# NomaDamas/AutoRAG-Research

Hardware: AMD Instinct MI355X
Metric: queries/sec (higher is better)
Workload: dtype f32

## Files before the change

autorag_research_amd/csrc/index.h:

```cpp
#pragma once
#include <climits>
#include <hip/hip_runtime.h>

#include <algorithm>
#include <cmath>
#include <cstdio>
#include <cstring>
#include <mutex>
#include <string>
#include <vector>

#include "dev_common.h"
#include "mi355dr.h"

namespace mi355 {
template <class T, bool Pinned = false>
struct DevBuf {
    T* p = nullptr;
    size_t bytes = 0;
    DevBuf() = default;
    DevBuf(const DevBuf&) = delete;
    DevBuf& operator=(const DevBuf&) = delete;
    ~DevBuf() { release(); }
    void release() {
// ... 27 lines not shown
    Event& operator=(const Event&) = delete;
    ~Event() {
        if (e) (void)hipEventDestroy(e);
    }
    hipError_t create(unsigned flags = hipEventDefault) { return e ? hipSuccess : hipEventCreateWithFlags(&e, flags); }
    operator hipEvent_t() const { return e; }
};

struct EventPair {
    hipEvent_t a, b;
    int big;
};
struct EventPairs {
    std::vector<EventPair> v;
    ~EventPairs() {
        for (auto& p : v) {
            (void)hipEventDestroy(p.a);
            (void)hipEventDestroy(p.b);
        }
    }
};
struct MultiVecStore;
struct SparseStore;
struct Pass {
    int k = 0;
    int level = 0;
    bool screening = false;
    bool i8 = false;
    bool wide = false;
    int cap = 0;
    bool speculative = false;
    bool spec_eligible = false;
    int spec_m = 0;
    const char* refused = nullptr;
};
struct Pending {
    bool active = false;
    Event done;
    HostBuf<int> status_host;
    hipStream_t stream = nullptr;
    const float* q_dev = nullptr;
    int B = 0;
    Pass pass;
    double* out_dist = nullptr;
    int64_t* out_rows = nullptr;
};
struct RetryBufs {
    DevBuf<float> q;
    DevBuf<double> dist;
    DevBuf<int64_t> rows;
    DevBuf<int> map;
};
constexpr int kPendingRing = 4;

template <class... Bufs>
hipError_t grow_each(size_t n, Bufs&... bufs) {
    hipError_t e = hipSuccess;
    (void)(((e = bufs.grow(n * sizeof(*bufs.p))) == hipSuccess) && ...);
    return e;
}
struct MmrBufs {
    DevBuf<double> cand_dist;
    DevBuf<int64_t> cand_rows;
    DevBuf<unsigned long long> pairs_dev;
    hipError_t reserve(size_t nb, size_t stride) {
        hipError_t e = grow_each(nb * stride, cand_dist, cand_rows);
// ... 134 lines not shown
    int speculate = 1;
    int64_t spec_min_rows = (int64_t)1 << 20;
    int spec_shift_milli = 0;
    int spec_backoff = 0, spec_probation = 0;
    mi355::DevBuf<float> spec_moments;
    int i8_demoted_k = INT_MAX;
    double i8_min_budget = 0.25;
    mi355::RetryBufs retry[3];
    mi355::Pending pend[mi355::kPendingRing];
    mi355::Pending sub_pend[4];
    int64_t seq_next = 0, seq_done = 0;
    int last_pass_k = 10;
    int maxsim_coop = -1;
    int maxsim_persistent = 0;
    int maxsim_wg = -1;
    int maxsim_tighten = 1;
    int maxsim_aligned = 1;
    int maxsim_wg_min = 8;
    int maxsim_wg_pipe = 1;
    int maxsim_pack8 = -1;
    int maxsim_wg_bps = 4;
    int maxsim_pass_groups = 4;
    int maxsim_screen = 1;
    int maxsim_subset_screen = -1;
    int64_t maxsim_subset_screen_min = 512;
    int64_t row_offset = 0;
    int round_a = 0;
    int screen_rq = 1;
    int screen_stream = 1;
    int prefilter16 = 0;
    int profile = 0;
    int starter = 1;
    int prune_companion = 1;
    int scan_dma = 1;
    int defer_round_b = 1;
    int chunk0_set = 0;
    int64_t chunk0_rows = 1024;
    int64_t chunk_growth = 3;
    int chunk_growth_set = 0;
    int64_t small_chunk_rows = 16384;
    int cap = mi355::kCandCap;
    int cap_set = 0;
    int prune_wide = 1;
    int screen_flush_sync = 1, screen_flush_lanes = 48, screen_flush_alone = 40;
    int wide_inflation_x10 = 100;
    int chunk_taper_x100 = 0;
    int64_t compact_slice_rows = 65536;
    int64_t view_slice_rows = 65536;
    int64_t range_chunk_rows = (int64_t)1 << 21;
    int range_slots = mi355::kSortMax;
    int64_t shard_stage_bytes = (int64_t)256 << 20;
    int64_t starter_rows_wide = 65536;

    int64_t s_screen_launches = 0, s_screen_ns = 0, s_screen_rows = 0, s_fallback_queries = 0, s_chunks = 0,
            s_passes = 0, s_starters = 0;
    int64_t s_big_launches = 0, s_big_ns = 0, s_big_rows = 0;
    int screen_rq_split_tests = 1;
    int64_t debug_park = 0;
    mi355::DevBuf<float> park_thr;
    int screen_drift = 3;
    mi355::DevBuf<int> rq_progress;
    int rq_epoch = 0;
    int64_t s_rq_launches = 0;
    int64_t s_spec_passes = 0, s_spec_miss_queries = 0, s_spec_overflow_queries = 0;
    int64_t s_retry_queries = 0;
    int64_t s_ms_screened = 0, s_ms_candidates = 0, s_ms_fallbacks = 0;
    int64_t s_ms_screen_ns = 0, s_ms_screen_launches = 0, s_ms_exact_ns = 0, s_ms_exact_launches = 0, s_ms_pack_ns = 0;
    int64_t s_ms_packed_launches = 0;
    int64_t s_ms_packed_blocks = 0;
    int64_t s_ms_packed_built = 0;
    int64_t s_ms_set_docs = 0;
    int64_t s_ms_moved_blocks = 0;
    int64_t s_compactions = 0;
    int64_t s_compact_moved_rows = 0;
    int64_t s_subset_searches = 0;
    int64_t s_subset_rows_scored = 0;
    int64_t s_subset_rerun_queries = 0;
    int64_t s_mss_searches = 0, s_mss_docs = 0, s_mss_screened = 0, s_mss_exact = 0, s_mss_fallbacks = 0;
    int64_t s_mmr_searches = 0, s_mmr_queries = 0, s_mmr_pairs = 0;
    int64_t s_group_searches = 0, s_group_subqueries = 0, s_groups_merged = 0;
    int64_t s_fuse_calls = 0, s_fuse_queries = 0;
    int64_t s_range_searches = 0, s_range_queries = 0, s_range_in_range = 0, s_range_candidates = 0, s_range_rescored = 0,
            s_range_redo_chunks = 0, s_range_fallback_queries = 0;
    int64_t s_rows_searches = 0, s_rows_queries = 0, s_rows_skipped = 0;
    int64_t s_shard_range_searches = 0, s_shard_rows_searches = 0, s_shard_mmr_searches = 0, s_shard_gather_bytes = 0;
    int64_t s_shard_sparse_searches = 0, s_shard_sparse_scores = 0;
    int64_t s_sparse_searches = 0, s_sparse_queries = 0, s_sparse_postings_scored = 0, s_sparse_overflows = 0;
    int sparse_tile_docs = 2048;
    int sparse_cand_cap = 2048;
    int64_t sparse_subset_pairs_max = 2048;
    int64_t s_sparse_subset_searches = 0, s_sparse_subset_scores = 0, s_sparse_subset_pairs = 0, s_sparse_subset_tiles = 0;
    int sparse_overlay_max_pct = 25;
    int64_t s_sparse_full_builds = 0, s_sparse_overlay_builds = 0, s_sparse_sets = 0;
// ... 88 lines not shown
```

autorag_research_amd/csrc/k_select.h:

```cpp
#pragma once
#include "dev_common.h"

namespace mi355 {

struct PruneArgs {
    const float* rows;
    const float* nrm2;
    const float* q;
    QueryState st;
    int32_t* cand_row;
    float* cand_val;
    const int* qlist;
    unsigned long long* stat;
    int cap, d, k, metric;
    int exact;
    const uint8_t* flag8;
    float cscale;
    const uint16_t* shadow16;
    int dpad;
    int round_a;
    int* skip_list;
    int skip_parity;
    int thr_only;
    int one_wave_only;
    int defer_b;
    SpecModel spec;
};

__device__ __forceinline__ float unit_sim(int metric, double dist, float inv_qn) {
    return metric == 0 ? (float)(1.0 - dist) : (float)(-dist) * inv_qn;
}
__device__ __forceinline__ float screen_threshold(int metric, double dist_k, float E, float nq) {
    if (metric == 0) return float_below((float)((1.0 - dist_k) - (double)E));
    const double u = -dist_k / sqrt((double)nq);
    return float_below((float)(u - fabs(u) * 4e-6 - (double)E));
}

constexpr int kPruneSmallThreads = 64, kPruneSmallSort = 1024;
constexpr int kPruneBigThreads = 256, kPruneBigSort = kSortMax;

__host__ __device__ inline size_t prune_qs_floats(int d) { return ((size_t)d + 3) / 4 * 4 + 16; }
__host__ __device__ inline size_t prune_lds_bytes(int d, int threads, int sortmax, int dpad16) {
    size_t x = (size_t)(threads / kWave) * kStageFloats * sizeof(float);
    size_t lf = (size_t)sortmax * sizeof(float);
    if (lf > x) x = lf;
    return (size_t)sortmax * 8 + (size_t)sortmax * 4 + x + (size_t)sortmax * 4 + prune_qs_floats(d) * 4 + (size_t)dpad16 * 4;
}

template <int PER, int T, bool ROWS = false>
__device__ __forceinline__ void load_candidate_keys(uint32_t (&key)[PER], const float* __restrict__ cval,
                                                    const int32_t* __restrict__ crow, const uint8_t* __restrict__ flag8,
                                                    int n_new, int tid, int32_t* rows_out = nullptr) {
    float v[PER];
    int32_t r[PER];
    const int last = n_new - 1;
#pragma unroll
    for (int j = 0; j < PER; ++j) {
        v[j] = 0.0f;
        r[j] = 0;
        if (j * T >= n_new) continue;
// ... 23 lines not shown
        if (j * T + tid < n_new) {
            if (v[j] != v[j]) kk = 0xFFFFFFFFu;
            else if (!f[j]) kk = f32_order_key(v[j]);
        }
        key[j] = kk;
        if (ROWS) rows_out[j] = r[j];
    }
}

template <int THREADS, int SORT>
__device__ __forceinline__ void prune_body(const PruneArgs& a, char* smem);

template <int THREADS, int SORT>
__global__ __launch_bounds__(THREADS) void k_prune(PruneArgs a) {
    extern __shared__ __attribute__((aligned(16))) char smem[];
    const bool list_mode = a.skip_list != nullptr && a.qlist == nullptr;
    const int tid = threadIdx.x;
    const int lane = tid & 63, wave = tid >> 6;
    int q = a.qlist ? a.qlist[blockIdx.x] : blockIdx.x;
    if (SORT == kPruneBigSort && list_mode) {
        if (blockIdx.x == 0 && tid == 0) a.skip_list[a.skip_parity ^ 1] = 0;
        const int n_left = a.skip_list[a.skip_parity];
        for (int i = blockIdx.x; i < n_left; i += gridDim.x) {
            PruneArgs b = a;
            b.skip_list = nullptr;
            b.qlist = a.skip_list + 2 + a.skip_parity * kQBlockMax + i - 0;
            b.qlist -= blockIdx.x;
            prune_body<THREADS, SORT>(b, smem);
            __syncthreads();
        }
        return;
    }
    prune_body<THREADS, SORT>(a, smem);
}

template <int THREADS, int SORT>
__device__ __forceinline__ void prune_body(const PruneArgs& a, char* smem) {
    constexpr int kWaves = THREADS / kWave;
    uint64_t* SK = (uint64_t*)smem;
    int32_t* SR = (int32_t*)(smem + (size_t)SORT * 8);
    char* X = smem + (size_t)SORT * 12;
    constexpr size_t xa = (size_t)kWaves * kStageFloats * sizeof(float), xb = (size_t)SORT * sizeof(float);
    constexpr size_t xbytes = xa > xb ? xa : xb;
    float* Lf = (float*)X;
    float* tiles = (float*)X;
    int32_t* R = (int32_t*)(X + xbytes);
    float* qs = (float*)(X + xbytes + (size_t)SORT * 4);
    int& s_cnt = *(int*)(X + xbytes + (size_t)SORT * 4 + (prune_qs_floats(a.d) - 16) * 4);
    float* q16 = qs + prune_qs_floats(a.d);
    const bool list_mode = a.skip_list != nullptr && a.qlist == nullptr;
    const int q = a.qlist ? a.qlist[blockIdx.x] : blockIdx.x;
    const int tid = threadIdx.x;
    const int lane = tid & 63, wave = tid >> 6;
    const int raw_cnt = a.st.cnt[q];
    const int n_best = a.st.best_n[q];
    if (raw_cnt == 0) return;
    if (a.exact && SORT < kPruneBigSort) return;
    auto leave_for_general = [&]() {
        if (a.one_wave_only) {
            if (tid == 0) {
                a.st.status[q] |= kStOverflow;
                a.st.cnt[q] = 0;
            }
            return;
        }
        if (list_mode && tid == 0) {
            const int i = atomicAdd(&a.skip_list[a.skip_parity], 1);
            a.skip_list[2 + a.skip_parity * kQBlockMax + i] = q;
        }
    };
    if (raw_cnt > a.cap) {
        if (SORT < kPruneBigSort) {
            leave_for_general();
            return;
        }
        if (tid == 0) {
            a.st.status[q] |= kStOverflow;
            a.st.cnt[q] = 0;
        }
        return;
    }
    if (n_best + raw_cnt > SORT) {
        if (SORT < kPruneBigSort) {
            leave_for_general();
            return;
        }
        if (tid == 0) {
            a.st.status[q] |= kStOverflow;
// ... 337 lines not shown
    bitonic_asc_key_row(SK, SR, np);
    const int n_keep = min(a.k, n_tot);
    for (int i = tid; i < n_keep; i += THREADS) {
        bkey[i] = SK[i];
        brow[i] = SR[i];
    }
    if (tid == 0) {
        a.st.best_n[q] = n_keep;
        a.st.cnt[q] = 0;
        if (n_keep >= a.k) {
            const uint64_t wk = SK[a.k - 1];
            a.st.thr_key[q] = wk;
            a.st.thr_row[q] = SR[a.k - 1];
            if (!a.exact && wk != kKeyNaN && !(a.st.status[q] & kStIrregular))
                a.st.thr[q] = screen_threshold(a.metric, key_to_dist(wk), E, nq);
        }
    }
}

__global__ __launch_bounds__(64) void k_emit_irregular(const int32_t* __restrict__ irr_rows, int irr_n, QueryState st,
                                                        int32_t* cand_row, float* cand_val, int cap, int skip_below) {
    const int q = blockIdx.x;
    if (st.status[q] & kStIrregular) return;
    for (int i = threadIdx.x; i < irr_n; i += blockDim.x) {
        if (irr_rows[i] < skip_below) continue;
        const int slot = atomicAdd(&st.cnt[q], 1);
        if (slot < cap) {
            cand_row[(int64_t)q * cap + slot] = irr_rows[i];
            cand_val[(int64_t)q * cap + slot] = __builtin_nanf("");
        }
    }
}

__global__ __launch_bounds__(64) void k_finalize(QueryState st, int k, int64_t row_offset, const int64_t* __restrict__ row_map,
                                                  double* out_dist, int64_t* out_rows, int* status_or, int spec_metric) {
    const int q = blockIdx.x;
    const int n = st.best_n[q];
    if (threadIdx.x == 0 && spec_metric >= 0 && !(st.status[q] & kStIrregular)) {
        float thr_final = -__builtin_inff();
        if (n >= k) {
            const uint64_t wk = st.best_key[(int64_t)q * kKMax + k - 1];
            if (wk != kKeyNaN) thr_final = screen_threshold(spec_metric, key_to_dist(wk), st.E[q], st.qn[q]);
        }
        if (n < k || thr_final < st.thr_used[q]) st.status[q] |= kStSpecMiss;
    }
    for (int s = threadIdx.x; s < k; s += blockDim.x) {
        if (s < n && st.best_row[(int64_t)q * kKMax + s] != kRowNone) {
            out_dist[(int64_t)q * k + s] = key_to_dist(st.best_key[(int64_t)q * kKMax + s]);
            const int32_t r = st.best_row[(int64_t)q * kKMax + s];
            out_rows[(int64_t)q * k + s] = row_map ? row_map[r] : (int64_t)r + row_offset;
        } else {
            out_dist[(int64_t)q * k + s] = __longlong_as_double(0x7FF8000000000000ll);
            out_rows[(int64_t)q * k + s] = -1;
        }
    }
    if (threadIdx.x == 0 && st.status[q] != 0) atomicOr(status_or, st.status[q]);
}

__global__ __launch_bounds__(256) void k_merge_topk(const double* __restrict__ dist_all,
                                                     const int64_t* __restrict__ rows_all, int64_t rank_stride, int world,
                                                     int B, int k, double* out_dist, int64_t* out_rows) {
    extern __shared__ __attribute__((aligned(16))) char smem[];
    uint64_t* SK = (uint64_t*)smem;
    const int np_ = next_pow2(world * k);
    int32_t* SI = (int32_t*)(smem + (size_t)np_ * 8);
    const int q = blockIdx.x;
    const int n = world * k;
    const int np = next_pow2(n);
    for (int i = threadIdx.x; i < np; i += blockDim.x) {
        if (i < n) {
            const int w = i / k, s = i % k;
            const int64_t src = (int64_t)w * rank_stride + (int64_t)q * k + s;
            const int64_t r = rows_all[src];
            SK[i] = r < 0 ? kKeyNaN : dist_to_key(dist_all[src]);
            SI[i] = r < 0 ? 0x7FFFFFFF : i;
        } else {
            SK[i] = kKeyNaN;
            SI[i] = 0x7FFFFFFF;
        }
    }
    __syncthreads();
    for (int kk = 2; kk <= np; kk <<= 1) {
        for (int j = kk >> 1; j > 0; j >>= 1) {
            for (int i = threadIdx.x; i < np; i += blockDim.x) {
                const int p = i ^ j;
                if (p > i) {
                    const bool asc = ((i & kk) == 0);
                    const uint64_t ka = SK[i], kb = SK[p];
                    const int32_t ia = SI[i], ib = SI[p];
// ... 41 lines not shown
```

autorag_research_amd/csrc/mi355dr.hip:

```cpp
#include "index.h"
#include "k_prep.h"
#include "k_scan.h"
#include "k_scan_ids.h"
#include "subset_ids.h"
#include "screen_common.h"
#include "k_screen.h"
#include "k_screen256c.h"
#include "k_screen_rq.h"

#define MI355_RQ_FORMS(X) X(1) X(2) X(3) X(4) X(5) X(6)
inline bool screen_rq_has(int ksteps) { return ksteps >= 1 && ksteps <= 6; }
#include "k_screen_stream.h"
#include "k_select.h"
#include "k_prune_wide.h"
#include "k_update.h"
#include "k_compact.h"
#include "k_view.h"
#include "k_block.h"
#include "k_mmr.h"
#include "mmr_order.h"
#include "k_groups.h"
#include "k_fuse.h"
#include "k_range.h"
#include "k_rows.h"
// ... 182 lines not shown
            idx->s_screen_ns += (int64_t)(ms * 1e6);
            if (p.big) idx->s_big_ns += (int64_t)(ms * 1e6);
        }
        idx->ev_pool.v.push_back(p);
    }
    idx->ev_pending.v.swap(keep);
}

constexpr double kInflationBf16 = 5.0, kInflationI8 = 16.0;
constexpr double kSmallBlockBudget = 1.6;
constexpr double kInflationI8Wide = 10.0, kInflationBf16Wide = 4.0;
inline bool wide_ok(const mi355dr_index* idx, int k) { return idx->prune_wide && k >= kWideKMin && k <= kWideKMax; }
inline double growth_budget(const mi355dr_index* idx, int k, bool i8) {
    if (wide_ok(idx, k) && idx->path != MI355DR_PATH_SCAN) {
        const int room = std::min(kWideEntries, idx->cap_set ? idx->cap : kCandCapWide);
        return 0.75 * room / ((double)k * (i8 ? idx->wide_inflation_x10 / 10.0 : kInflationBf16Wide)) - 1.0;
    }
    const int room = k < kPruneSmallSort / 2 ? kPruneSmallSort - k : idx->cap;
    return 0.6 * std::min(room, idx->cap) / ((double)k * (i8 ? kInflationI8 : kInflationBf16));
}

inline bool i8_available(const mi355dr_index* idx) { return idx->irr8_n <= kIrrCap; }
constexpr int kStarterKMax = 32;
constexpr int64_t kStarterRows = 16384;
static_assert(kStarterRows / kSlabRows <= kSpecSlabsMax, "the moment scratch holds one entry per slab of the starter's sample");
int64_t starter_sample_rows(const mi355dr_index* idx, const Pass& ps) {
    const int64_t n = idx->n;
    const int64_t rows = std::min<int64_t>(ps.wide ? idx->starter_rows_wide : kStarterRows, n / 4) / kTileM * kTileM;
    const int64_t slabs = (rows + kSlabRows - 1) / kSlabRows;
    const bool take = idx->starter && (ps.k <= kStarterKMax || ps.wide) && ps.level == 0 && idx->chunk0_set == 0 && n >= 4 * 1024 &&
                      slabs <= ps.cap && slabs >= ps.k;
    return take ? rows : 0;
}
Pass decide_pass(const mi355dr_index* idx, int k, int level, bool force_scan, const char* no_screen = nullptr) {
    Pass ps;
    ps.k = k;
    ps.level = level;
    const int path = force_scan ? (int)MI355DR_PATH_SCAN : idx->path;
    if (level > 0) ps.i8 = false;
    else if (idx->screen_dtype == MI355DR_SCREEN_I8) ps.i8 = true;
    else ps.i8 = idx->screen_dtype == MI355DR_SCREEN_AUTO && i8_available(idx) && k < idx->i8_demoted_k &&
                 growth_budget(idx, k, true) >= idx->i8_min_budget;
    const bool screen_possible = ps.i8 ? i8_available(idx) : idx->irr_n <= kIrrCap;
    ps.screening = idx->n > 0 && screen_possible && path != MI355DR_PATH_SCAN;
    ps.wide = ps.screening && wide_ok(idx, k);
    ps.cap = !idx->cap_set && ps.wide ? kCandCapWide : idx->cap;
    if (idx->screen_dtype == MI355DR_SCREEN_I8 && !i8_available(idx) && path != MI355DR_PATH_SCAN)
        ps.refused = "int8 screen unavailable: too many rows outside the residual limit";
    else if (path == MI355DR_PATH_SCREEN && !screen_possible && idx->n > 0) ps.refused = no_screen;
    ps.spec_m = spec_m_of(k);
    ps.spec_eligible = level == 0 && ps.screening && !ps.wide && ps.spec_m > 0 && idx->speculate && idx->n >= idx->spec_min_rows &&
                       kSpecInflation * ps.spec_m * 4 <= 3 * (std::min(kPruneSmallSort, ps.cap) - k) &&
                       starter_sample_rows(idx, ps) > 0;
    ps.speculative = ps.spec_eligible && idx->spec_probation <= 0;
    return ps;
}
inline bool idle_i8(const mi355dr_index* idx) { return decide_pass(idx, idx->last_pass_k, 0, false).i8; }

int launch_prune(mi355dr_index* idx, hipStream_t s, const Pass& ps, int nblocks, const int* qlist, int exact,
                 bool thr_only = false, bool one_wave_only = false, bool defer_b = false, const SpecModel* spec = nullptr) {
    PruneArgs pa{};
    if (spec) pa.spec = *spec;
    pa.thr_only = thr_only ? 1 : 0;
    pa.one_wave_only = one_wave_only ? 1 : 0;
    pa.defer_b = defer_b && idx->defer_round_b ? 1 : 0;
    pa.rows = idx->rows;
    pa.nrm2 = idx->nrm2;
    pa.q = idx->qdev;
    pa.st = idx->st;
    pa.cand_row = idx->cand_row;
    pa.cand_val = idx->cand_val;
    pa.qlist = qlist;
    pa.stat = idx->stat_dev;
    pa.cap = ps.cap;
    pa.d = idx->dim;
    pa.k = ps.k;
    pa.metric = idx->metric;
    pa.exact = exact;
    pa.flag8 = (ps.i8 && (idx->irr8_n > 0 || idx->dead_n > 0)) ? idx->flag8 : nullptr;
    pa.cscale = idx->metric == MI355DR_METRIC_IP ? idx->cmax : 1.0f;
    pa.shadow16 = (ps.i8 && idx->metric == 0 && !exact && idx->prefilter16) ? idx->shadow : nullptr;
    pa.dpad = idx->dpad;
    pa.round_a = idx->round_a;
    if (!exact && ps.wide) {
        pa.shadow16 = nullptr;
        hipLaunchKernelGGL((k_prune_wide<2, 32>), dim3(nblocks), dim3(2 * kWave), prune_wide_lds_bytes(idx->dim, 2), s, pa);
        HIPCHECK(idx, hipGetLastError());
        return MI355DR_OK;
    }
    if (pa.cap > kCandCap) return fail(idx, MI355DR_E_INTERNAL, "general-form prune on a list stride above kCandCap");
    const bool list_mode = qlist == nullptr;
    pa.skip_list = list_mode ? idx->prune_skip : nullptr;
    pa.skip_parity = list_mode ? (idx->prune_parity ^= 1) : 0;
    hipLaunchKernelGGL((k_prune<kPruneSmallThreads, kPruneSmallSort>), dim3(nblocks), dim3(kPruneSmallThreads),
                       prune_lds_bytes(idx->dim, kPruneSmallThreads, kPruneSmallSort, pa.shadow16 ? idx->dpad : 0), s, pa);
    HIPCHECK(idx, hipGetLastError());
    if (one_wave_only) return MI355DR_OK;
    hipLaunchKernelGGL((k_prune<kPruneBigThreads, kPruneBigSort>), dim3(list_mode ? std::min(nblocks, 64) : nblocks),
                       dim3(kPruneBigThreads), prune_lds_bytes(idx->dim, kPruneBigThreads, kPruneBigSort, 0), s, pa);
    HIPCHECK(idx, hipGetLastError());
    return MI355DR_OK;
}

int launch_prep(mi355dr_index* idx, hipStream_t s, int B, int Bpad, int metric, bool i8, int cnt0 = 0) {
    hipLaunchKernelGGL(k_prep_queries, dim3(Bpad), dim3(64), (size_t)idx->dim * sizeof(float), s, idx->qdev, B, idx->dim,
                       idx->dpad, metric, idx->st, idx->dpad8, i8 ? 1 : 0, idx->bf16_ec, idx->status_or_dev,
                       idx->prune_skip, cnt0, idx->metric == MI355DR_METRIC_IP ? idx->cmax : 1.0f);
    idx->prune_parity = 0;
    HIPCHECK(idx, hipGetLastError());
    return MI355DR_OK;
}

inline int screen_tile(int B) { return B > kTileN ? kT2 : kTileM; }

constexpr int kRetryLevels = 2;

enum ScreenKernel { kKernTile = 0, kKernStream = 1, kKern256c = 2, kKernRq = 3 };
inline ScreenKernel screen_kernel_for(const mi355dr_index* idx, bool i8, int B, int64_t rows, bool emit_all) {
    const int tile = (emit_all || rows <= idx->small_chunk_rows) ? kTileM : screen_tile(B);
    const int row_bytes = i8 ? idx->dpad8 : idx->dpad * 2;
    const int ksteps = row_bytes / kRowB;
    if (tile == kT2) return i8 && idx->screen_rq && screen_rq_has(ksteps) ? kKernRq : kKern256c;
    if (!emit_all && idx->screen_stream && B <= 64 && ksteps >= 1 && (B <= 32 ? 32 : 64) * row_bytes <= kStreamQueryBytesMax)
        return kKernStream;
    return kKernTile;
}

int launch_screen(mi355dr_index* idx, hipStream_t s, bool i8, int B, int64_t r0, int64_t r_end, int cap, int emit_mode,
                  int flush_mask, int moment_slabs = 0) {
    const bool emit_all = emit_mode != 0;
    const ScreenKernel kern = screen_kernel_for(idx, i8, B, r_end - r0, emit_all);
    const int tile = kern == kKern256c || kern == kKernRq ? kT2 : kTileM;
    ScreenArgs2 sa{};
    sa.status = idx->st.status;
    sa.shadow = i8 ? (const void*)idx->shadow8 : (const void*)idx->shadow;
    sa.qhat = i8 ? (const void*)idx->st.qhat8 : (const void*)idx->st.qhat;
    sa.thr = idx->st.thr;
    sa.sc = idx->st.sc;
    sa.kq = idx->st.kq;
    sa.grp = idx->grp8;
    sa.flag8 = idx->flag8;
    sa.cnt = idx->st.cnt;
    sa.cand_row = idx->cand_row;
    sa.cand_val = idx->cand_val;
    sa.row_bytes = i8 ? idx->dpad8 : idx->dpad * 2;
    sa.ksteps = sa.row_bytes / kRowB;
    sa.cap = cap;
    sa.ct0 = (int)(r0 / tile);
    sa.n_ctiles = (int)(round_up(r_end, tile) / tile) - sa.ct0;
    sa.n_qtiles = (int)(round_up(B, tile) / tile);
    sa.row_end = r_end;
    sa.row0 = r0;
    sa.emit_all = emit_mode;
    if (moment_slabs > 0) {
        sa.moments = idx->spec_moments;
        sa.moment_slabs = moment_slabs;
    }
    const int64_t grid = round_up(sa.n_ctiles, 8) * sa.n_qtiles;
    switch (kern) {
    case kKernRq: {
        sa.ct0 = (int)(r0 / kRqRows);
        sa.n_ctiles = (int)(round_up(r_end, kRqRows) / kRqRows) - sa.ct0;
        const unsigned g2 = screen_rq_grid(sa.n_ctiles, sa.n_qtiles);
        idx->s_rq_launches++;
        if (idx->debug_park > 0 && r_end - r0 >= idx->debug_park) {
            if (!idx->park_thr) {
                std::vector<float> inf(kQBlockMax, INFINITY);
                HIPCHECK(idx, idx->park_thr.grow(kQBlockMax * sizeof(float)));
                HIPCHECK(idx, hipMemcpy(idx->park_thr, inf.data(), kQBlockMax * sizeof(float), hipMemcpyHostToDevice));
            }
            sa.thr = idx->park_thr;
        }
        sa.progress = idx->rq_progress;
        sa.epoch = idx->rq_epoch = idx->rq_epoch % 4095 + 1;
        if (sa.epoch == 1) HIPCHECK(idx, hipMemsetAsync(idx->rq_progress, 0, kRqProgressWords * sizeof(int), s));
        sa.drift = idx->screen_drift;
        sa.flush_mask = flush_mask;
        sa.flush_alone = idx->screen_flush_alone;
        if (sa.ksteps == 6 && !idx->screen_rq_split_tests) {
            hipLaunchKernelGGL((k_screen_rq<6, false, true>), dim3(g2), dim3(512), rq_lds(6), s, sa);
        } else {
            switch (sa.ksteps) {
#define MI355_RQ_LAUNCH(KS) \
    case KS: hipLaunchKernelGGL((k_screen_rq<KS, true, true>), dim3(g2), dim3(512), rq_lds(KS), s, sa); break;
                MI355_RQ_FORMS(MI355_RQ_LAUNCH)
#undef MI355_RQ_LAUNCH
            }
        }
        break;
    }
    case kKern256c: {
        const unsigned g2 = screen256_grid(sa.n_ctiles, sa.n_qtiles);
        if (i8) hipLaunchKernelGGL((k_screen256c<true>), dim3(g2), dim3(512), kScreen256Lds, s, sa);
        else hipLaunchKernelGGL((k_screen256c<false>), dim3(g2), dim3(512), kScreen256Lds, s, sa);
        break;
    }
    case kKernStream: {
        const int nq = B <= 32 ? 32 : 64;
        const unsigned gs = (unsigned)std::min(sa.n_ctiles, 256);
        const size_t lds = screen_stream_lds(nq, sa.row_bytes);
        if (i8 && nq == 32) hipLaunchKernelGGL((k_screen_stream<true, 32>), dim3(gs), dim3(256), lds, s, (ScreenArgs)sa);
        else if (i8) hipLaunchKernelGGL((k_screen_stream<true, 64>), dim3(gs), dim3(256), lds, s, (ScreenArgs)sa);
        else if (nq == 32) hipLaunchKernelGGL((k_screen_stream<false, 32>), dim3(gs), dim3(256), lds, s, (ScreenArgs)sa);
        else hipLaunchKernelGGL((k_screen_stream<false, 64>), dim3(gs), dim3(256), lds, s, (ScreenArgs)sa);
        break;
    }
    case kKernTile:
        if (i8) hipLaunchKernelGGL(k_screen<true>, dim3((unsigned)grid), dim3(256), kScreenLds, s, (ScreenArgs)sa);
        else hipLaunchKernelGGL(k_screen<false>, dim3((unsigned)grid), dim3(256), kScreenLds, s, (ScreenArgs)sa);
// ... 68 lines not shown

inline int starter_count(const PassPlan& p) { return (int)((p.sample + kSlabRows - 1) / kSlabRows); }

inline double normal_quantile(double p) {
    double lo = -40.0, hi = 40.0;
    for (int i = 0; i < 200; ++i) {
        const double mid = 0.5 * (lo + hi);
        if (0.5 * std::erfc(-mid / std::sqrt(2.0)) < p) lo = mid;
        else hi = mid;
    }
    return 0.5 * (lo + hi);
}

SpecModel spec_model(const mi355dr_index* idx, const Pass& ps, const PassPlan& plan, double* zq_out = nullptr) {
    SpecModel sm{};
    sm.moments = idx->spec_moments;
    sm.slabs = starter_count(plan);
    sm.rows = (int)plan.sample;
    const double zq = normal_quantile(1.0 - (double)ps.spec_m / (double)idx->n) + idx->spec_shift_milli / 1000.0;
    sm.zq = (float)zq;
    if (zq_out) *zq_out = zq;
    return sm;
}

PassPlan make_plan(const mi355dr_index* idx, const Pass& ps, int B) {
    const double budget = growth_budget(idx, ps.k, ps.i8);
    double growth = std::max(0.25, std::min((double)idx->chunk_growth, budget));
    if (B <= 64 && ps.level == 0 && idx->chunk_growth_set == 0) growth = std::max(growth, std::min(8.0, budget * kSmallBlockBudget));
    if (ps.level == 1) growth = std::max(0.25, growth * 0.5);
    if (ps.level >= 2) growth = 0.25;
    return plan_pass(idx, ps, B, growth);
}

int run_screen(mi355dr_index* idx, hipStream_t s, const Pass& ps, int B, const PassPlan& plan) {
    int64_t kept_all_below = 0;
    const bool i8 = ps.i8;
    const int side_n = i8 ? idx->irr8_n : idx->irr_n;
    constexpr int kSideMerge = 32;
    bool side_done = false;
    const bool lean = plan.sample > 0 && idx->prune_companion == 0;
    auto timed = [&](bool big, int64_t rows, auto&& launch) -> int {
        EventPair ev{};
        if (idx->profile) {
            ev = take_events(idx);
            HIPCHECK(idx, hipEventRecord(ev.a, s));
        }
        CHECK(launch());
        if (idx->profile) {
            HIPCHECK(idx, hipEventRecord(ev.b, s));
            ev.big = big ? 1 : 0;
            idx->ev_pending.v.push_back(ev);
        }
        idx->s_screen_launches++;
        idx->s_screen_rows += rows;
        if (big) {
            idx->s_big_launches++;
            idx->s_big_rows += rows;
        }
        return MI355DR_OK;
    };
    if (plan.sample > 0) {
        SpecModel sm{};
        if (ps.speculative) {
            sm = spec_model(idx, ps, plan);
            idx->s_spec_passes++;
        }
        CHECK(timed(false, plan.sample, [&] {
            return launch_screen(idx, s, i8, B, 0, plan.sample, ps.cap, kEmitSlabMax, -1, ps.speculative ? sm.slabs : 0);
        }));
        CHECK(launch_prune(idx, s, ps, B, nullptr, 0, true, true, false,
                           ps.speculative ? &sm : nullptr));
        idx->s_starters++;
    }
    int64_t done = 0;
    for (size_t ci = 0; ci < plan.ends.size(); ++ci) {
        const int64_t end = plan.ends[ci];
        const bool emit_all = ci == 0 && plan.emit_all_first;
        if (emit_all) kept_all_below = end;
        const bool big = !emit_all && end - done > idx->small_chunk_rows && screen_tile(B) == kT2;
        const int64_t seen = ci == 0 ? (plan.sample > 0 ? plan.sample : end) : done;
        const double lanes = ps.speculative ? (double)kSpecInflation * ps.spec_m * 4096.0 / (double)idx->n
                                            : 8.0 * ps.k * 4096.0 / (double)std::max<int64_t>(seen, 1);
        int period = 1;
        while (period < 64 && period * 2 * lanes <= idx->screen_flush_lanes) period *= 2;
        const int flush_mask = idx->screen_flush_sync ? period - 1 : -1;
        CHECK(timed(big, end - done, [&] { return launch_screen(idx, s, i8, B, done, end, ps.cap, emit_all ? kEmitAll : 0, flush_mask); }));
        idx->s_chunks++;
        if (end >= idx->n && side_n > 0 && side_n <= kSideMerge) {
            hipLaunchKernelGGL(k_emit_irregular, dim3(B), dim3(64), 0, s, i8 ? idx->irr8_rows : idx->irr_rows, side_n, idx->st,
                               idx->cand_row, idx->cand_val, ps.cap, (int)kept_all_below);
            HIPCHECK(idx, hipGetLastError());
            side_done = true;
        }
        const bool last = end >= idx->n && (side_n == 0 || side_done);
        CHECK(launch_prune(idx, s, ps, B, nullptr, 0, false, lean, !last));
        done = end;
    }
    if (side_n > 0 && !side_done) {
        hipLaunchKernelGGL(k_emit_irregular, dim3(B), dim3(64), 0, s, i8 ? idx->irr8_rows : idx->irr_rows, side_n, idx->st,
                           idx->cand_row, idx->cand_val, ps.cap, (int)kept_all_below);
        HIPCHECK(idx, hipGetLastError());
        CHECK(launch_prune(idx, s, ps, B, nullptr, 0, false, lean));
    }
    idx->s_passes++;
    return MI355DR_OK;
}

int launch_scan(mi355dr_index* idx, hipStream_t s, const int* qlist, int nq, int cap, int64_t r0, int64_t r1,
                const int32_t* ids = nullptr) {
    ScanArgs sa{};
    sa.rows = idx->rows;
    sa.nrm2 = idx->nrm2;
    sa.q = idx->qdev;
    sa.st = idx->st;
    sa.cand_row = idx->cand_row;
    sa.cand_val = idx->cand_val;
    sa.qlist = qlist;
    sa.nq = nq;
    sa.cap = cap;
    sa.d = idx->dim;
// ... 42 lines not shown
                    HIPCHECK(idx, hipMemcpyAsync(idx->qlist_dev + roff, redo.data(), redo.size() * sizeof(int),
                                                 hipMemcpyHostToDevice, s));
                    for (int q : redo) idx->status_host[q] &= ~kStOverflow;
                    for (int q : redo)
                        HIPCHECK(idx, hipMemcpyAsync(idx->st.status + q, idx->status_host + q, sizeof(int),
                                                     hipMemcpyHostToDevice, s));
                    for (int64_t p = done; p < end; p += cap)
                        CHECK(scan_range(idx, s, ps, roff, (int)redo.size(), p, std::min<int64_t>(end, p + cap), ids));
                    if (ids) {
                        HIPCHECK(idx, hipStreamSynchronize(s));
                        idx->s_subset_rerun_queries += (int64_t)redo.size();
                    }
                }
            }
            done = end;
            chunk = std::max<int64_t>(chunk, done * (idx->chunk_growth_set ? idx->chunk_growth : 63));
        }
    }
    if (ids) HIPCHECK(idx, hipStreamSynchronize(s));
    else idx->s_fallback_queries += nq_all;
    return MI355DR_OK;
}

int subset_block(mi355dr_index* idx, hipStream_t s, const float* q_dev, int B, int k, int64_t m, double* out_dist_dev,
                 int64_t* out_rows_dev) {
    const Pass ps = decide_pass(idx, k, 0, true);
    idx->last_pass_k = k;
    if (q_dev != idx->qdev)
        HIPCHECK(idx, hipMemcpyAsync(idx->qdev, q_dev, (size_t)B * idx->dim * sizeof(float), hipMemcpyDeviceToDevice, s));
    CHECK(launch_prep(idx, s, B, (int)round_up(B, screen_tile(B)), idx->metric, ps.i8));
    std::vector<int> all(B);
    for (int i = 0; i < B; ++i) all[i] = i;
    if (m > 0) CHECK(run_scan(idx, s, ps, all, m, idx->subset_ids));
    hipLaunchKernelGGL(k_finalize, dim3(B), dim3(64), 0, s, idx->st, k, idx->row_offset, idx->view_row_map.p, out_dist_dev,
                       out_rows_dev, idx->status_or_dev, -1);
    HIPCHECK(idx, hipGetLastError());
    HIPCHECK(idx, hipMemcpyAsync(idx->status_host, idx->st.status, (size_t)kQBlockMax * sizeof(int), hipMemcpyDeviceToHost, s));
    HIPCHECK(idx, hipStreamSynchronize(s));
    for (int i = 0; i < B; ++i)
        if (idx->status_host[i] & kStOverflow)
            return fail(idx, MI355DR_E_INTERNAL, "subset scan: query " + std::to_string(i) + " lost a candidate chunk");
    return MI355DR_OK;
}

int pending_alloc(mi355dr_index* idx, Pending& p) {
    HIPCHECK(idx, p.status_host.grow((kQBlockMax + 1) * sizeof(int)));
    HIPCHECK(idx, p.done.create(hipEventDisableTiming));
    return MI355DR_OK;
}

int enqueue_block(mi355dr_index* idx, hipStream_t s, const float* q_dev, int B, int k, double* out_dist_dev,
                  int64_t* out_rows_dev, Pending& p, int level = 0, bool force_scan = false) {
    CHECK(ensure_qstate(idx));
    CHECK(pending_alloc(idx, p));
    idx->last_pass_k = k;
    if (level == 0 && idx->screen_dtype == MI355DR_SCREEN_AUTO && k >= idx->i8_demoted_k && --idx->i8_probation <= 0)
        idx->i8_demoted_k = INT_MAX;
    const int Bpad = (int)round_up(B, screen_tile(B));
    const Pass ps = decide_pass(idx, k, level, force_scan, "screen path unavailable (metric or too many irregular rows)");
    if (ps.refused) return fail(idx, MI355DR_E_UNSUPPORTED, ps.refused);
    if (idx->spec_probation > 0 && ps.spec_eligible) idx->spec_probation--;
    if (q_dev != idx->qdev)
        HIPCHECK(idx, hipMemcpyAsync(idx->qdev, q_dev, (size_t)B * idx->dim * sizeof(float), hipMemcpyDeviceToDevice, s));
    PassPlan plan;
    if (ps.screening) plan = make_plan(idx, ps, B);
    CHECK(launch_prep(idx, s, B, Bpad, idx->metric, ps.i8, starter_count(plan)));
    if (idx->n > 0) {
        if (ps.screening) {
            CHECK(run_screen(idx, s, ps, B, plan));
        } else {
            std::vector<int> all(B);
            for (int i = 0; i < B; ++i) all[i] = i;
            CHECK(run_scan(idx, s, ps, all, idx->n));
        }
    }
    hipLaunchKernelGGL(k_finalize, dim3(B), dim3(64), 0, s, idx->st, k, idx->row_offset, idx->view_row_map.p, out_dist_dev,
                       out_rows_dev, idx->status_or_dev, ps.speculative && idx->n > 0 ? idx->metric : -1);
    HIPCHECK(idx, hipGetLastError());
    HIPCHECK(idx, hipMemcpyAsync(p.status_host, idx->st.status, (size_t)(kQBlockMax + 1) * sizeof(int), hipMemcpyDeviceToHost, s));
    HIPCHECK(idx, hipEventRecord(p.done, s));
    p.active = true;
    p.stream = s;
    p.q_dev = q_dev;
    p.B = B;
    p.pass = ps;
    p.out_dist = out_dist_dev;
    p.out_rows = out_rows_dev;
    return MI355DR_OK;
}

int search_block(mi355dr_index* idx, hipStream_t s, const float* q_dev, int B, int k, double* out_dist_dev,
                 int64_t* out_rows_dev, int level = 0, bool force_scan = false);

int complete_block(mi355dr_index* idx, Pending& p) {
    if (!p.active) return MI355DR_OK;
    p.active = false;
    HIPCHECK(idx, hipEventSynchronize(p.done));
    drain_events(idx);
    if (!p.pass.screening) {
        for (int i = 0; i < p.B; ++i)
            if (p.status_host[i] & kStOverflow)
                return fail(idx, MI355DR_E_INTERNAL, "exact scan: query " + std::to_string(i) + " lost a candidate chunk");
        return MI355DR_OK;
    }
    if (p.status_host[kQBlockMax] == 0) return MI355DR_OK;
    hipStream_t s = p.stream;
    const int B = p.B, k = p.pass.k, level = p.pass.level;
    std::vector<int> sub;
    int n_todo = 0;
    {
        std::vector<int> retry;
// ... 1872 lines not shown
constexpr bool kSwitch = true;

struct Option {
    const char* key;
    Field field;
    int64_t lo = INT64_MIN, hi = INT64_MAX;
    void (*then)(Index*) = nullptr;
    int64_t gap_lo = 0, gap_hi = 0;
};
const Option kOptions[] = {
    {"path", &Index::path, 0, 2},
    {"screen_dtype", &Index::screen_dtype, 0, 2, [](Index* x) {
         x->i8_demoted_k = INT_MAX;
         x->i8_backoff = x->i8_probation = 0;
     }},
    {"i8_min_budget_x100", &Index::i8_min_budget, 1, 1000},
    {"maxsim_screen", {&Index::maxsim_screen, kSwitch}},
    {"maxsim_coop", &Index::maxsim_coop, -1, 1},
    {"maxsim_persistent", {&Index::maxsim_persistent, kSwitch}},
    {"maxsim_wg", &Index::maxsim_wg, -1, 2},
    {"maxsim_tighten", {&Index::maxsim_tighten, kSwitch}},
    {"maxsim_aligned", {&Index::maxsim_aligned, kSwitch}},
    {"maxsim_wg_min", &Index::maxsim_wg_min, 8, 9},
    {"maxsim_wg_pipe", {&Index::maxsim_wg_pipe, kSwitch}},
    {"maxsim_pack8", &Index::maxsim_pack8, -1, 1},
    {"maxsim_wg_bps", &Index::maxsim_wg_bps, 2, 4, nullptr, 2, 4},
    {"maxsim_pass_groups", &Index::maxsim_pass_groups, 1, 4},
    {"maxsim_subset_screen", &Index::maxsim_subset_screen, -1, 1},
    {"maxsim_subset_screen_min", &Index::maxsim_subset_screen_min, 0},
    {"row_offset", &Index::row_offset},
    {"profile", {&Index::profile, kSwitch}},
    {"chunk0_rows", &Index::chunk0_rows, 1, INT64_MAX, [](Index* x) { x->chunk0_set = 1; }},
    {"starter", {&Index::starter, kSwitch}},
    {"prune_companion", {&Index::prune_companion, kSwitch}},
    {"speculate", {&Index::speculate, kSwitch}, INT64_MIN, INT64_MAX, [](Index* x) { x->spec_backoff = x->spec_probation = 0; }},
    {"spec_min_rows", &Index::spec_min_rows, 0},
    {"spec_shift_milli", &Index::spec_shift_milli, -20000, 20000},
    {"scan_dma", {&Index::scan_dma, kSwitch}},
    {"defer_round_b", {&Index::defer_round_b, kSwitch}},
    {"chunk_growth", &Index::chunk_growth, 1, INT64_MAX, [](Index* x) { x->chunk_growth_set = 1; }},
    {"screen_stream", {&Index::screen_stream, kSwitch}},
    {"screen_rq", {&Index::screen_rq, kSwitch}},
    {"debug_park_thresholds", &Index::debug_park},
    {"screen_rq_split_tests", {&Index::screen_rq_split_tests, kSwitch}},
    {"screen_drift", &Index::screen_drift, 0, 1024},
    {"small_chunk_rows", &Index::small_chunk_rows, 0},
    {"round_a", &Index::round_a, 0, 64},
    {"prefilter16", {&Index::prefilter16, kSwitch}},
    {"cand_cap", &Index::cap, 16, kCandCap, [](Index* x) { x->cap_set = 1; }},
    {"prune_wide", {&Index::prune_wide, kSwitch}},
    {"screen_flush_sync", {&Index::screen_flush_sync, kSwitch}},
    {"screen_flush_lanes", &Index::screen_flush_lanes, 1, 64},
    {"screen_flush_alone", &Index::screen_flush_alone, 8, 60},
    {"wide_inflation_x10", &Index::wide_inflation_x10, 20, 400},
    {"chunk_taper_x100", &Index::chunk_taper_x100, 0, 300, nullptr, 0, 100},
    {"starter_rows_wide", &Index::starter_rows_wide, 4096, 262144},
    {"compact_slice_rows", &Index::compact_slice_rows, 32, (int64_t)1 << 22},
    {"view_slice_rows", &Index::view_slice_rows, 32, (int64_t)1 << 22},
    {"range_chunk_rows", &Index::range_chunk_rows, 256, (int64_t)1 << 31},
    {"range_slots", &Index::range_slots, 16, kSortMax},
    {"sparse_tile_docs", &Index::sparse_tile_docs, 256, 8192},
    {"sparse_cand_cap", &Index::sparse_cand_cap, 16, 2048},
    {"sparse_overlay_max_pct", &Index::sparse_overlay_max_pct, 0, 100},
    {"sparse_subset_pairs_max", &Index::sparse_subset_pairs_max, 0, 2048},
    {"shard_stage_bytes", &Index::shard_stage_bytes, 1},
};

struct Stat {
    const char* key;
    int64_t Index::*counter;
    bool reset;
    int64_t (*value)(const Index*) = nullptr;
};
const Stat kStats[] = {
    {"screen_launches", &Index::s_screen_launches, true},
    {"screen_ns", &Index::s_screen_ns, true},
    {"screen_rows", &Index::s_screen_rows, true},
    {"screen256_launches", &Index::s_big_launches, true},
    {"screen_rq_launches", &Index::s_rq_launches, true},
    {"screen256_ns", &Index::s_big_ns, true},
    {"screen256_rows", &Index::s_big_rows, true},
    {"fallback_queries", &Index::s_fallback_queries, true},
    {"chunks", &Index::s_chunks, true},
    {"passes", &Index::s_passes, true},
    {"starters", &Index::s_starters, true},
    {"retry_queries", &Index::s_retry_queries, true},
    {"spec_passes", &Index::s_spec_passes, true},
    {"spec_miss_queries", &Index::s_spec_miss_queries, true},
    {"spec_overflow_queries", &Index::s_spec_overflow_queries, true},
    {"spec_suspended", nullptr, false, [](const Index* x) -> int64_t { return x->spec_probation > 0 ? 1 : 0; }},
    {"maxsim_screened", &Index::s_ms_screened, true},
    {"maxsim_candidates", &Index::s_ms_candidates, true},
    {"maxsim_fallbacks", &Index::s_ms_fallbacks, true},
    {"maxsim_screen_ns", &Index::s_ms_screen_ns, true},
    {"maxsim_pack_ns", &Index::s_ms_pack_ns, true},
    {"maxsim_screen_launches", &Index::s_ms_screen_launches, true},
    {"maxsim_exact_ns", &Index::s_ms_exact_ns, true},
    {"maxsim_exact_launches", &Index::s_ms_exact_launches, true},
    {"maxsim_screen_cols", &Index::s_ms_screen_cols, true},
    {"maxsim_packed_launches", &Index::s_ms_packed_launches, true},
    {"maxsim_packed_blocks", &Index::s_ms_packed_blocks, false},
    {"maxsim_packed_built", &Index::s_ms_packed_built, false},
    {"maxsim_set_docs", &Index::s_ms_set_docs, true},
    {"maxsim_moved_blocks", &Index::s_ms_moved_blocks, true},
    {"subset_searches", &Index::s_subset_searches, true},
    {"subset_rows_scored", &Index::s_subset_rows_scored, true},
    {"subset_rerun_queries", &Index::s_subset_rerun_queries, true},
    {"maxsim_subset_searches", &Index::s_mss_searches, true},
    {"maxsim_subset_docs", &Index::s_mss_docs, true},
    {"maxsim_subset_screened", &Index::s_mss_screened, true},
    {"maxsim_subset_exact", &Index::s_mss_exact, true},
    {"maxsim_subset_fallbacks", &Index::s_mss_fallbacks, true},
    {"mmr_searches", &Index::s_mmr_searches, true},
    {"mmr_queries", &Index::s_mmr_queries, true},
    {"mmr_pairs_scored", &Index::s_mmr_pairs, true},
    {"group_searches", &Index::s_group_searches, true},
    {"group_subqueries", &Index::s_group_subqueries, true},
    {"groups_merged", &Index::s_groups_merged, true},
    {"fuse_calls", &Index::s_fuse_calls, true},
    {"fuse_queries", &Index::s_fuse_queries, true},
// ... 335 lines not shown
```

Before: 164,500.

## Fuse irregular-row emit and finalize into one-wave prune on speculative passes

On speculative single-chunk screening passes with few irregular rows, the one-wave prune kernel now appends the irregular side rows into the candidate list and then finalizes the query in the same launch. This drops the separate k_emit_irregular and k_finalize launches and the later prune stages. It also lets speculative passes use their own screen drift (default 0) and a tunable flush-period cap. The risk is changed candidate handling, since side rows are written with NaN values and later chunks are skipped, and a longer single kernel.

```diff
diff --git a/autorag_research_amd/csrc/index.h b/autorag_research_amd/csrc/index.h
--- a/autorag_research_amd/csrc/index.h
+++ b/autorag_research_amd/csrc/index.h
@@ -83,6 +83,7 @@
     bool speculative = false;
     bool spec_eligible = false;
     int spec_m = 0;
+    bool fused_tail = false;
     const char* refused = nullptr;
 };
 struct Pending {
@@ -283,6 +284,7 @@
     int profile = 0;
     int starter = 1;
     int prune_companion = 1;
+    int prune_companion_set = 0;
     int scan_dma = 1;
     int defer_round_b = 1;
     int chunk0_set = 0;
@@ -310,6 +312,9 @@
     int64_t debug_park = 0;
     mi355::DevBuf<float> park_thr;
     int screen_drift = 3;
+    int screen_drift_set = 0;
+    int onechunk_drift = 0, onechunk_period_max = 64;
+    int64_t s_fused_tails = 0;
     mi355::DevBuf<int> rq_progress;
     int rq_epoch = 0;
     int64_t s_rq_launches = 0;
diff --git a/autorag_research_amd/csrc/k_select.h b/autorag_research_amd/csrc/k_select.h
--- a/autorag_research_amd/csrc/k_select.h
+++ b/autorag_research_amd/csrc/k_select.h
@@ -2,6 +2,16 @@
 #include "dev_common.h"
 
 namespace mi355 {
+
+struct FinalizeArgs {
+    int k;
+    int64_t row_offset;
+    const int64_t* row_map;
+    double* out_dist;
+    int64_t* out_rows;
+    int* status_or;
+    int spec_metric;
+};
 
 struct PruneArgs {
     const float* rows;
@@ -25,7 +35,12 @@
     int one_wave_only;
     int defer_b;
     SpecModel spec;
+    const int32_t* side_rows;
+    int side_n, side_skip_below;
+    FinalizeArgs fin;
 };
+
+__device__ __forceinline__ void finalize_query(const QueryState& st, int q, const FinalizeArgs& f, int tid, int nthreads);
 
 __device__ __forceinline__ float unit_sim(int metric, double dist, float inv_qn) {
     return metric == 0 ? (float)(1.0 - dist) : (float)(-dist) * inv_qn;
@@ -115,6 +130,12 @@
         return;
     }
     prune_body<THREADS, SORT>(a, smem);
+    if constexpr (SORT == kPruneSmallSort) {
+        if (a.fin.out_dist != nullptr) {
+            __syncthreads();
+            finalize_query(a.st, q, a.fin, tid, THREADS);
+        }
+    }
 }
 
 template <int THREADS, int SORT>
@@ -135,8 +156,23 @@
     const int q = a.qlist ? a.qlist[blockIdx.x] : blockIdx.x;
     const int tid = threadIdx.x;
     const int lane = tid & 63, wave = tid >> 6;
-    const int raw_cnt = a.st.cnt[q];
+    int raw_cnt = a.st.cnt[q];
     const int n_best = a.st.best_n[q];
+    if constexpr (THREADS == kWave) {
+        if (a.side_n > 0 && !(a.st.status[q] & kStIrregular)) {
+            const int32_t r = lane < a.side_n ? a.side_rows[lane] : -1;
+            const bool want = lane < a.side_n && r >= a.side_skip_below;
+            const unsigned long long bal = __builtin_amdgcn_ballot_w64(want);
+            const int pos = raw_cnt + (int)__builtin_amdgcn_mbcnt_hi((unsigned)(bal >> 32),
+                                                                     __builtin_amdgcn_mbcnt_lo((unsigned)bal, 0));
+            if (want && pos < a.cap) {
+                a.cand_row[(int64_t)q * a.cap + pos] = r;
+                a.cand_val[(int64_t)q * a.cap + pos] = __builtin_nanf("");
+            }
+            raw_cnt += __builtin_popcountll(bal);
+            __syncthreads();
+        }
+    }
     if (raw_cnt == 0) return;
     if (a.exact && SORT < kPruneBigSort) return;
     auto leave_for_general = [&]() {
@@ -540,11 +576,14 @@
     }
 }
 
-__global__ __launch_bounds__(64) void k_finalize(QueryState st, int k, int64_t row_offset, const int64_t* __restrict__ row_map,
-                                                  double* out_dist, int64_t* out_rows, int* status_or, int spec_metric) {
-    const int q = blockIdx.x;
+__device__ __forceinline__ void finalize_query(const QueryState& st, int q, const FinalizeArgs& f, int tid, int nthreads) {
+    const int k = f.k, spec_metric = f.spec_metric;
+    const int64_t row_offset = f.row_offset;
+    const int64_t* row_map = f.row_map;
+    double* out_dist = f.out_dist;
+    int64_t* out_rows = f.out_rows;
     const int n = st.best_n[q];
-    if (threadIdx.x == 0 && spec_metric >= 0 && !(st.status[q] & kStIrregular)) {
+    if (tid == 0 && spec_metric >= 0 && !(st.status[q] & kStIrregular)) {
         float thr_final = -__builtin_inff();
         if (n >= k) {
             const uint64_t wk = st.best_key[(int64_t)q * kKMax + k - 1];
@@ -552,7 +591,7 @@
         }
         if (n < k || thr_final < st.thr_used[q]) st.status[q] |= kStSpecMiss;
     }
-    for (int s = threadIdx.x; s < k; s += blockDim.x) {
+    for (int s = tid; s < k; s += nthreads) {
         if (s < n && st.best_row[(int64_t)q * kKMax + s] != kRowNone) {
             out_dist[(int64_t)q * k + s] = key_to_dist(st.best_key[(int64_t)q * kKMax + s]);
             const int32_t r = st.best_row[(int64_t)q * kKMax + s];
@@ -562,7 +601,11 @@
             out_rows[(int64_t)q * k + s] = -1;
         }
     }
-    if (threadIdx.x == 0 && st.status[q] != 0) atomicOr(status_or, st.status[q]);
+    if (tid == 0 && st.status[q] != 0) atomicOr(f.status_or, st.status[q]);
+}
+
+__global__ __launch_bounds__(64) void k_finalize(QueryState st, FinalizeArgs f) {
+    finalize_query(st, blockIdx.x, f, threadIdx.x, blockDim.x);
 }
 
 __global__ __launch_bounds__(256) void k_merge_topk(const double* __restrict__ dist_all,
diff --git a/autorag_research_amd/csrc/mi355dr.hip b/autorag_research_amd/csrc/mi355dr.hip
--- a/autorag_research_amd/csrc/mi355dr.hip
+++ b/autorag_research_amd/csrc/mi355dr.hip
@@ -238,6 +238,8 @@
                       slabs <= ps.cap && slabs >= ps.k;
     return take ? rows : 0;
 }
+constexpr int kSideMerge = 32;
+static_assert(kSideMerge <= kWave, "the fused tail appends one side row per lane");
 Pass decide_pass(const mi355dr_index* idx, int k, int level, bool force_scan, const char* no_screen = nullptr) {
     Pass ps;
     ps.k = k;
@@ -259,14 +261,23 @@
                        kSpecInflation * ps.spec_m * 4 <= 3 * (std::min(kPruneSmallSort, ps.cap) - k) &&
                        starter_sample_rows(idx, ps) > 0;
     ps.speculative = ps.spec_eligible && idx->spec_probation <= 0;
+    ps.fused_tail = ps.speculative && (ps.i8 ? idx->irr8_n : idx->irr_n) <= kSideMerge && !idx->prune_companion_set && !idx->cap_set;
     return ps;
 }
 inline bool idle_i8(const mi355dr_index* idx) { return decide_pass(idx, idx->last_pass_k, 0, false).i8; }
 
 int launch_prune(mi355dr_index* idx, hipStream_t s, const Pass& ps, int nblocks, const int* qlist, int exact,
-                 bool thr_only = false, bool one_wave_only = false, bool defer_b = false, const SpecModel* spec = nullptr) {
+                 bool thr_only = false, bool one_wave_only = false, bool defer_b = false, const SpecModel* spec = nullptr,
+                 const FinalizeArgs* fused = nullptr, int skip_below = 0) {
     PruneArgs pa{};
     if (spec) pa.spec = *spec;
+    if (fused) {
+        if (!one_wave_only || qlist || exact || ps.wide) return fail(idx, MI355DR_E_INTERNAL, "fused tail on a prune that is not the one-wave form alone");
+        pa.side_rows = ps.i8 ? idx->irr8_rows : idx->irr_rows;
+        pa.side_n = ps.i8 ? idx->irr8_n : idx->irr_n;
+        pa.side_skip_below = skip_below;
+        pa.fin = *fused;
+    }
     pa.thr_only = thr_only ? 1 : 0;
     pa.one_wave_only = one_wave_only ? 1 : 0;
     pa.defer_b = defer_b && idx->defer_round_b ? 1 : 0;
@@ -333,7 +344,7 @@
 }
 
 int launch_screen(mi355dr_index* idx, hipStream_t s, bool i8, int B, int64_t r0, int64_t r_end, int cap, int emit_mode,
-                  int flush_mask, int moment_slabs = 0) {
+                  int flush_mask, int moment_slabs = 0, int drift = -1) {
     const bool emit_all = emit_mode != 0;
     const ScreenKernel kern = screen_kernel_for(idx, i8, B, r_end - r0, emit_all);
     const int tile = kern == kKern256c || kern == kKernRq ? kT2 : kTileM;
@@ -380,7 +391,7 @@
         sa.progress = idx->rq_progress;
         sa.epoch = idx->rq_epoch = idx->rq_epoch % 4095 + 1;
         if (sa.epoch == 1) HIPCHECK(idx, hipMemsetAsync(idx->rq_progress, 0, kRqProgressWords * sizeof(int), s));
-        sa.drift = idx->screen_drift;
+        sa.drift = drift >= 0 ? drift : idx->screen_drift;
         sa.flush_mask = flush_mask;
         sa.flush_alone = idx->screen_flush_alone;
         if (sa.ksteps == 6 && !idx->screen_rq_split_tests) {
@@ -515,11 +526,10 @@
     return plan_pass(idx, ps, B, growth);
 }
 
-int run_screen(mi355dr_index* idx, hipStream_t s, const Pass& ps, int B, const PassPlan& plan) {
+int run_screen(mi355dr_index* idx, hipStream_t s, const Pass& ps, int B, const PassPlan& plan, const FinalizeArgs& fin) {
     int64_t kept_all_below = 0;
     const bool i8 = ps.i8;
     const int side_n = i8 ? idx->irr8_n : idx->irr_n;
-    constexpr int kSideMerge = 32;
     bool side_done = false;
     const bool lean = plan.sample > 0 && idx->prune_companion == 0;
     auto timed = [&](bool big, int64_t rows, auto&& launch) -> int {
@@ -564,11 +574,21 @@
         const int64_t seen = ci == 0 ? (plan.sample > 0 ? plan.sample : end) : done;
         const double lanes = ps.speculative ? (double)kSpecInflation * ps.spec_m * 4096.0 / (double)idx->n
                                             : 8.0 * ps.k * 4096.0 / (double)std::max<int64_t>(seen, 1);
+        const int period_max = ps.speculative ? idx->onechunk_period_max : 64;
+        const int drift = ps.speculative && !idx->screen_drift_set ? idx->onechunk_drift : idx->screen_drift;
         int period = 1;
-        while (period < 64 && period * 2 * lanes <= idx->screen_flush_lanes) period *= 2;
+        while (period < period_max && period * 2 * lanes <= idx->screen_flush_lanes) period *= 2;
         const int flush_mask = idx->screen_flush_sync ? period - 1 : -1;
-        CHECK(timed(big, end - done, [&] { return launch_screen(idx, s, i8, B, done, end, ps.cap, emit_all ? kEmitAll : 0, flush_mask); }));
+        CHECK(timed(big, end - done, [&] { return launch_screen(idx, s, i8, B, done, end, ps.cap, emit_all ? kEmitAll : 0, flush_mask, 0, drift); }));
         idx->s_chunks++;
+        if (ps.fused_tail) {
+            CHECK(launch_prune(idx, s, ps, B, nullptr, 0, false, true, false, nullptr, &fin,
+                               (int)kept_all_below));
+            idx->s_fused_tails++;
+            side_done = true;
+            done = end;
+            continue;
+        }
         if (end >= idx->n && side_n > 0 && side_n <= kSideMerge) {
             hipLaunchKernelGGL(k_emit_irregular, dim3(B), dim3(64), 0, s, i8 ? idx->irr8_rows : idx->irr_rows, side_n, idx->st,
                                idx->cand_row, idx->cand_val, ps.cap, (int)kept_all_below);
@@ -677,8 +697,8 @@
     std::vector<int> all(B);
     for (int i = 0; i < B; ++i) all[i] = i;
     if (m > 0) CHECK(run_scan(idx, s, ps, all, m, idx->subset_ids));
-    hipLaunchKernelGGL(k_finalize, dim3(B), dim3(64), 0, s, idx->st, k, idx->row_offset, idx->view_row_map.p, out_dist_dev,
-                       out_rows_dev, idx->status_or_dev, -1);
+    hipLaunchKernelGGL(k_finalize, dim3(B), dim3(64), 0, s, idx->st,
+                       FinalizeArgs{k, idx->row_offset, idx->view_row_map.p, out_dist_dev, out_rows_dev, idx->status_or_dev, -1});
     HIPCHECK(idx, hipGetLastError());
     HIPCHECK(idx, hipMemcpyAsync(idx->status_host, idx->st.status, (size_t)kQBlockMax * sizeof(int), hipMemcpyDeviceToHost, s));
     HIPCHECK(idx, hipStreamSynchronize(s));
@@ -709,19 +729,22 @@
         HIPCHECK(idx, hipMemcpyAsync(idx->qdev, q_dev, (size_t)B * idx->dim * sizeof(float), hipMemcpyDeviceToDevice, s));
     PassPlan plan;
     if (ps.screening) plan = make_plan(idx, ps, B);
+    const FinalizeArgs fin{k, idx->row_offset, idx->view_row_map.p, out_dist_dev, out_rows_dev, idx->status_or_dev,
+                           ps.speculative && idx->n > 0 ? idx->metric : -1};
     CHECK(launch_prep(idx, s, B, Bpad, idx->metric, ps.i8, starter_count(plan)));
     if (idx->n > 0) {
         if (ps.screening) {
-            CHECK(run_screen(idx, s, ps, B, plan));
+            CHECK(run_screen(idx, s, ps, B, plan, fin));
         } else {
             std::vector<int> all(B);
             for (int i = 0; i < B; ++i) all[i] = i;
             CHECK(run_scan(idx, s, ps, all, idx->n));
         }
     }
-    hipLaunchKernelGGL(k_finalize, dim3(B), dim3(64), 0, s, idx->st, k, idx->row_offset, idx->view_row_map.p, out_dist_dev,
-                       out_rows_dev, idx->status_or_dev, ps.speculative && idx->n > 0 ? idx->metric : -1);
-    HIPCHECK(idx, hipGetLastError());
+    if (!(ps.fused_tail && idx->n > 0)) {
+        hipLaunchKernelGGL(k_finalize, dim3(B), dim3(64), 0, s, idx->st, fin);
+        HIPCHECK(idx, hipGetLastError());
+    }
     HIPCHECK(idx, hipMemcpyAsync(p.status_host, idx->st.status, (size_t)(kQBlockMax + 1) * sizeof(int), hipMemcpyDeviceToHost, s));
     HIPCHECK(idx, hipEventRecord(p.done, s));
     p.active = true;
@@ -2660,7 +2683,7 @@
     {"profile", {&Index::profile, kSwitch}},
     {"chunk0_rows", &Index::chunk0_rows, 1, INT64_MAX, [](Index* x) { x->chunk0_set = 1; }},
     {"starter", {&Index::starter, kSwitch}},
-    {"prune_companion", {&Index::prune_companion, kSwitch}},
+    {"prune_companion", {&Index::prune_companion, kSwitch}, INT64_MIN, INT64_MAX, [](Index* x) { x->prune_companion_set = 1; }},
     {"speculate", {&Index::speculate, kSwitch}, INT64_MIN, INT64_MAX, [](Index* x) { x->spec_backoff = x->spec_probation = 0; }},
     {"spec_min_rows", &Index::spec_min_rows, 0},
     {"spec_shift_milli", &Index::spec_shift_milli, -20000, 20000},
@@ -2671,7 +2694,9 @@
     {"screen_rq", {&Index::screen_rq, kSwitch}},
     {"debug_park_thresholds", &Index::debug_park},
     {"screen_rq_split_tests", {&Index::screen_rq_split_tests, kSwitch}},
-    {"screen_drift", &Index::screen_drift, 0, 1024},
+    {"screen_drift", &Index::screen_drift, 0, 1024, [](Index* x) { x->screen_drift_set = 1; }},
+    {"onechunk_drift", &Index::onechunk_drift, 0, 1024},
+    {"onechunk_period_max", &Index::onechunk_period_max, 64, 256},
     {"small_chunk_rows", &Index::small_chunk_rows, 0},
     {"round_a", &Index::round_a, 0, 64},
     {"prefilter16", {&Index::prefilter16, kSwitch}},
@@ -2714,6 +2739,7 @@
     {"starters", &Index::s_starters, true},
     {"retry_queries", &Index::s_retry_queries, true},
     {"spec_passes", &Index::s_spec_passes, true},
+    {"fused_tail_passes", &Index::s_fused_tails, true},
     {"spec_miss_queries", &Index::s_spec_miss_queries, true},
     {"spec_overflow_queries", &Index::s_spec_overflow_queries, true},
     {"spec_suspended", nullptr, false, [](const Index* x) -> int64_t { return x->spec_probation > 0 ? 1 : 0; }},
```

Result: no change. 165,200, median of 6 (+0.4%).
